# divortio/divortio-lz4

Measured on NVIDIA B200. Metric: lz4_block_roundtrip_throughput, higher is better.
Workload: dtype u8

## Files before the change

divortio-lz4_b200/csrc/api_ctx.inc:

```
namespace {

constexpr int kWarpsFresh16 = 7;
constexpr int kWarpsGeneric32 = 3;
constexpr int kWarpsDecode = 8;
constexpr int kJdGroupEvent = 112;
constexpr int kGtabRegions = 5;
constexpr uint32_t kMaxSplitBlocks = 1u << 20;

struct Buf {
    void *p = nullptr;
    size_t cap = 0;
};

class CopyPool {
  public:
    explicit CopyPool(int threads) {
        for (int i = 0; i < threads; ++i) workers_.emplace_back([this] { run(); });
    }
    ~CopyPool() {
        { std::lock_guard<std::mutex> g(m_); stop_ = true; }
        cv_.notify_all();
        for (std::thread &t : workers_) t.join();
    }
    void copy(void *dst, const void *src, size_t n) {
// ... 50 lines not shown
    std::atomic<size_t> next_{0};
};
constexpr int kSumSlots = 32;
constexpr int kStageSlots = 4;
constexpr size_t kStageBytes = 16u << 20;

}

struct dlz4_ctx {
    int device = 0;
    int sm_count = 0;
    cudaStream_t stream = nullptr, side = nullptr, copy_in = nullptr, copy_out = nullptr;
    cudaStream_t lanes[4] = {};
    uint64_t chunk_bytes = 64ull << 20;
    int n_lanes = 3;
    cudaEvent_t evp[128] = {};
    cudaEvent_t ev0 = nullptr, ev1 = nullptr, ev_side = nullptr, ev_fork = nullptr;
    uint32_t *d_counter = nullptr;
    uint32_t *d_land = nullptr;
    uint32_t *h_one = nullptr;
    uint64_t seg_overlap_min_bytes = 64ull << 20;
    uint32_t *d_hash = nullptr;
    uint64_t *d_total = nullptr;
    int32_t *d_table = nullptr;
    int split = 1;
    bool pw = true;
    int pw_sleep = 200;
    int pw_lead = 7;
    Buf rec;
    uint32_t *d_nrec = nullptr;
    int hybrid = 1;
    int hy_grid = 0;
    int hy_active = 0;
    uint16_t *d_gtabs = nullptr;
    Buf work, comp, seg, out, meta, aux, pin;
    Buf fb_frames, fb_blocks, fb_comp, fb_io;
    std::string last_error;
    uint64_t frame_pipe_min_bytes = 32ull << 20;
    uint64_t jump_min_bytes = 256ull << 10;
    uint64_t seg_min_bytes = 256ull << 10;
    uint32_t seg_jobs = 0, seg_reruns = 0, seg_rounds = 0;
    uint64_t launches = 0;
    float last_ms = 0.f;
    int64_t k_seg_kib = -1, k_seg_warm_kib = -1, k_seg_unit_kib = -1;
    int k_seg_group = -1, k_seg_no_chase = 0, k_jd_unit_mib = 0, k_jd_serial_scan = 0, k_jd_no_overlap = 0, k_debug = 0;
    CopyPool *pool = nullptr;
    int copy_threads = 0;
    uint8_t *stage[kStageSlots] = {};
    cudaEvent_t stage_ev[kStageSlots] = {};
    bool stage_busy[kStageSlots] = {};
    cudaStream_t sum_stream[kSumSlots] = {};
    uint32_t *h_sum = nullptr;
    int probe = 0;
    cudaEvent_t evq[3] = {};
    const uint8_t *res_in = nullptr, *res_out = nullptr;
    uint64_t res_in_len = 0, res_out_len = 0, res_body_len = 0;
};

namespace {

#define CK(call)                                                                                      \
    do {                                                                                              \
        cudaError_t e_ = (call);                                                                      \
        if (e_ != cudaSuccess) {                                                                      \
            char m_[512];                                                                             \
            snprintf(m_, sizeof m_, "%s failed: %s (%s:%d)", #call, cudaGetErrorString(e_), __FILE__, __LINE__); \
            ctx->last_error = m_;                                                                     \
            return DLZ4_E_CUDA;                                                                       \
        }                                                                                             \
    } while (0)

#define CKS(expr)                       \
    do {                                \
        int s_ = (expr);                \
        if (s_ != DLZ4_OK) return s_;   \
    } while (0)

int reserve(dlz4_ctx *ctx, Buf &b, size_t bytes) {
    bytes = (bytes + 255) & ~(size_t)255;
    if (bytes + 256 <= b.cap) return DLZ4_OK;
    if (b.p) CK(cudaFree(b.p));
    b.p = nullptr; b.cap = 0;
    size_t want = bytes + 256;
    CK(cudaMalloc(&b.p, want));
    b.cap = want;
    return DLZ4_OK;
}

int reserve_pinned(dlz4_ctx *ctx, Buf &b, size_t bytes) {
    if (bytes <= b.cap) return DLZ4_OK;
    if (b.p) CK(cudaFreeHost(b.p));
    b.p = nullptr; b.cap = 0;
    CK(cudaMallocHost(&b.p, bytes));
    b.cap = bytes;
    return DLZ4_OK;
}

inline cudaStream_t pick(dlz4_ctx *ctx, void *stream) { return stream ? (cudaStream_t)stream : ctx->stream; }

bool is_pageable(const void *p) {
    cudaPointerAttributes a;
    if (cudaPointerGetAttributes(&a, p) != cudaSuccess) { cudaGetLastError(); return true; }
    return a.type == cudaMemoryTypeUnregistered;
}

int stage_init(dlz4_ctx *ctx) {
    if (ctx->stage[0]) return DLZ4_OK;
// ... 76 lines not shown
```

divortio-lz4_b200/csrc/api_launch.inc:

```
int compress_segmented(dlz4_ctx *ctx, const uint8_t *d_work, int64_t start, int64_t total, int64_t B, uint32_t n, bool linked,
                       const int32_t *init_table, uint8_t *d_comp, const uint64_t *d_coff, uint32_t *d_clen, cudaStream_t st,
                       int32_t *final_table = nullptr, const uint32_t *landed = nullptr, int32_t land_origin = 0,
                       uint32_t land_shift = 0);

int launch_compress(dlz4_ctx *ctx, const uint8_t *src, const uint64_t *src_off, const uint32_t *src_len, uint32_t n,
                    uint32_t max_len, const uint8_t *prefix, uint32_t prefix_len, const int32_t *init_table, uint8_t *dst,
                    const uint64_t *dst_off, uint32_t *comp_len, cudaStream_t st, uint32_t *counter = nullptr, bool dense = false) {
    if (n == 0) return DLZ4_OK;
    if (!counter) counter = ctx->d_counter;
    CK(cudaMemsetAsync(counter, 0, sizeof(uint32_t), st));
    if (init_table == nullptr) { prefix = nullptr; prefix_len = 0; }
    if (max_len <= 65536 && prefix_len == 0 && init_table == nullptr && ctx->split && n <= kMaxSplitBlocks) {
        const size_t region = (size_t)(counter - ctx->d_counter) % kGtabRegions;
        const uint64_t rstride = (uint64_t)max_len / 4 + 2;
        const size_t region_bytes = (((size_t)n * rstride * 8) * 9 / 8 + 255) & ~(size_t)255;
        if (ctx->rec.cap < region_bytes * kGtabRegions + 256) {
            CK(cudaDeviceSynchronize());
            CKS(reserve(ctx, ctx->rec, std::max(region_bytes, (size_t)ctx->rec.cap / kGtabRegions) * kGtabRegions));
        }
        const size_t per_region = ((ctx->rec.cap - 256) / kGtabRegions) & ~(size_t)255;
        uint64_t *recs = (uint64_t *)((uint8_t *)ctx->rec.p + region * per_region);
        uint32_t *nrec = ctx->d_nrec + region * (size_t)kMaxSplitBlocks;
        if (ctx->probe) CK(cudaEventRecord(ctx->evq[0], st));
        if (ctx->pw) {
            const int grid = (int)std::min<uint64_t>(n, (uint64_t)ctx->sm_count);
            const uint32_t lead = (uint32_t)ctx->pw_lead, ns = (uint32_t)ctx->pw_sleep;
            k_parse_pw<<<grid, kPwThreads, kPwSmemBytes, st>>>(src, src_off, src_len, n, recs, rstride, nrec, counter, lead, ns);
        } else
        {
            const int grid = (int)std::min<uint64_t>((n + kWarpsFresh16 - 1) / kWarpsFresh16, (uint64_t)ctx->sm_count);
            k_parse_fresh16<kWarpsFresh16><<<grid, kWarpsFresh16 * 32, kWarpsFresh16 * kHashEntries * 2, st>>>(
                src, src_off, src_len, n, recs, rstride, nrec, counter);
        }
        if (ctx->probe) CK(cudaEventRecord(ctx->evq[1], st));
        CK(cudaMemsetAsync(counter, 0, sizeof(uint32_t), st));
        const int egrid = (int)std::min<uint64_t>((n + kWarpsDecode - 1) / kWarpsDecode, (uint64_t)ctx->sm_count * 8);
        k_encode_blocks<kWarpsDecode><<<egrid, kWarpsDecode * 32, 0, st>>>(src, src_off, src_len, n, recs, rstride, nrec, dst, dst_off,
                                                                            comp_len, counter);
        if (ctx->probe) CK(cudaEventRecord(ctx->evq[2], st));
        ctx->launches++;
    } else if (max_len <= 65536 && prefix_len == 0 && init_table == nullptr && ctx->hybrid) {
        const size_t region = (size_t)(counter - ctx->d_counter) % kGtabRegions;
        const int grid = (int)std::min<uint64_t>(dense ? (n + kHyWarps - 1) / kHyWarps : n, (uint64_t)ctx->hy_grid);
        uint32_t active = dense ? (uint32_t)kHyWarps : (uint32_t)std::min<uint64_t>((n + grid - 1) / grid, (uint64_t)kHyWarps);
        if (ctx->hy_active) active = std::min<uint32_t>(active, (uint32_t)ctx->hy_active);
        k_compress_fresh16h<<<grid, kHyWarps * 32, kHySmemBytes, st>>>(
            src, src_off, src_len, n, dst, dst_off, comp_len, counter,
            ctx->d_gtabs + region * (size_t)ctx->hy_grid * kHyGlWarps * kHashEntries, active);
    } else if (max_len <= 4096 && prefix_len > 0 && init_table != nullptr && ctx->hybrid && prefix_len < 0x7FFF0000u) {
        const size_t region = (size_t)(counter - ctx->d_counter) % kGtabRegions;
        const int grid = (int)std::min<uint64_t>(dense ? (n + kHyWarps - 1) / kHyWarps : n, (uint64_t)ctx->hy_grid);
        const uint32_t active = dense ? (uint32_t)kHyWarps : (uint32_t)std::min<uint64_t>((n + grid - 1) / grid, (uint64_t)kHyWarps);
        k_compress_overlay<<<grid, kHyWarps * 32, kHySmemBytes, st>>>(
            src, src_off, src_len, n, prefix, prefix_len, init_table, dst, dst_off, comp_len, counter,
            ctx->d_gtabs + region * (size_t)ctx->hy_grid * kHyGlWarps * kHashEntries, active);
    } else {
        if (max_len > 65536 && prefix_len == 0 && init_table == nullptr && n <= 65536) {
            std::vector<uint64_t> off(n);
            std::vector<uint32_t> len(n);
            CK(cudaMemcpyAsync(off.data(), src_off, (size_t)n * 8, cudaMemcpyDeviceToHost, st));
            CK(cudaMemcpyAsync(len.data(), src_len, (size_t)n * 4, cudaMemcpyDeviceToHost, st));
            CK(cudaStreamSynchronize(st));
            const uint64_t B = len[0];
            bool uniform = B > 65536 && (B & (B - 1)) == 0 && off[0] + (uint64_t)n * B < 0x7FFFFFF0ull;
            for (uint32_t i = 0; uniform && i < n; ++i)
                uniform = off[i] == off[0] + (uint64_t)i * B && (len[i] == B || (i + 1 == n && len[i] <= B && len[i] > 0));
            if (uniform) {
                const int64_t total = (int64_t)(n - 1) * (int64_t)B + len[n - 1];
                return compress_segmented(ctx, src, (int64_t)off[0], total, (int64_t)B, n, false, nullptr, dst, dst_off, comp_len, st);
            }
        }
        const int grid = (int)std::min<uint64_t>((n + kWarpsGeneric32 - 1) / kWarpsGeneric32, (uint64_t)ctx->sm_count);
        k_compress_generic32<kWarpsGeneric32><<<grid, kWarpsGeneric32 * 32, kWarpsGeneric32 * (kHashEntries * 4 + kRingBytes), st>>>(
            src, src_off, src_len, n, prefix, prefix_len, init_table, dst, dst_off, comp_len, counter);
    }
    ctx->launches++;
    CK(cudaGetLastError());
    return DLZ4_OK;
}

int launch_decompress(dlz4_ctx *ctx, const uint8_t *src, const uint64_t *src_off, const uint32_t *src_len, uint32_t n,
                      uint8_t *dst, const uint64_t *dst_off, const uint32_t *dst_cap, const uint8_t *dict, uint32_t dict_len,
                      int hist_frame, const uint8_t *stored, uint32_t *out_len, uint8_t *status, cudaStream_t st,
                      uint32_t *counter = nullptr) {
    if (n == 0) return DLZ4_OK;
    if (!counter) counter = ctx->d_counter;
    CK(cudaMemsetAsync(counter, 0, sizeof(uint32_t), st));
    const int grid = hist_frame ? 1 : (int)std::min<uint64_t>((n + kWarpsDecode - 1) / kWarpsDecode, (uint64_t)ctx->sm_count * 8);
    if (dict_len)
        k_decompress_blocks<kWarpsDecode, true><<<grid, hist_frame ? 32 : kWarpsDecode * 32, 0, st>>>(src, src_off, src_len, n, dst, dst_off, dst_cap,
                                                                                                      dict, dict_len, hist_frame, stored, out_len, status, counter);
    else
// ... 25 lines not shown
```

divortio-lz4_b200/csrc/api_lifecycle.inc:

```
int dlz4_init(int device, dlz4_ctx **out) {
    if (!out) return DLZ4_E_INVALID_ARG;
    *out = nullptr;
    dlz4_ctx *ctx = new dlz4_ctx();
    ctx->device = device;
    *out = ctx;
    int count = 0;
    CK(cudaGetDeviceCount(&count));
    if (device < 0 || device >= count) { ctx->last_error = "no such CUDA device"; return DLZ4_E_CUDA; }
    CK(cudaSetDevice(device));
    cudaDeviceProp prop;
    CK(cudaGetDeviceProperties(&prop, device));
    ctx->sm_count = prop.multiProcessorCount;
    CK(cudaStreamCreateWithFlags(&ctx->stream, cudaStreamNonBlocking));
    CK(cudaStreamCreateWithFlags(&ctx->side, cudaStreamNonBlocking));
    CK(cudaStreamCreateWithFlags(&ctx->copy_in, cudaStreamNonBlocking));
    CK(cudaStreamCreateWithFlags(&ctx->copy_out, cudaStreamNonBlocking));
    for (cudaEvent_t &e : ctx->evp) CK(cudaEventCreateWithFlags(&e, cudaEventDisableTiming));
    CK(cudaEventCreate(&ctx->ev0));
    CK(cudaEventCreate(&ctx->ev1));
    for (cudaEvent_t &e : ctx->evq) CK(cudaEventCreate(&e));
    CK(cudaEventCreateWithFlags(&ctx->ev_side, cudaEventDisableTiming));
    CK(cudaEventCreateWithFlags(&ctx->ev_fork, cudaEventDisableTiming));
    for (cudaStream_t &l : ctx->lanes) CK(cudaStreamCreateWithFlags(&l, cudaStreamNonBlocking));
    if (const char *e = getenv("DLZ4_SEG_KIB")) ctx->k_seg_kib = std::max(0, atoi(e));
    if (const char *e = getenv("DLZ4_SEG_WARM_KIB")) ctx->k_seg_warm_kib = std::max(0, atoi(e));
    if (const char *e = getenv("DLZ4_SEG_UNIT_KIB")) ctx->k_seg_unit_kib = std::max(0, atoi(e));
    if (const char *e = getenv("DLZ4_SEG_GROUP")) ctx->k_seg_group = std::max(0, atoi(e));
    ctx->k_seg_no_chase = getenv("DLZ4_SEG_NO_CHASE") != nullptr;
    if (const char *e = getenv("DLZ4_JD_UNIT_MIB")) ctx->k_jd_unit_mib = std::max(1, atoi(e));
    ctx->k_jd_serial_scan = getenv("DLZ4_JD_SERIAL_SCAN") != nullptr;
    ctx->k_jd_no_overlap = getenv("DLZ4_JD_NO_OVERLAP") != nullptr;
    ctx->k_debug = getenv("DLZ4_DEBUG") != nullptr;
    if (const char *e = getenv("DLZ4_CHUNK_MIB")) ctx->chunk_bytes = (uint64_t)std::max(1, atoi(e)) << 20;
    if (const char *e = getenv("DLZ4_LANES")) ctx->n_lanes = std::min(4, std::max(1, atoi(e)));
    if (const char *e = getenv("DLZ4_COPY_THREADS")) ctx->copy_threads = std::min(64, std::max(1, atoi(e)));
    CK(cudaMalloc(&ctx->d_counter, 64));
    CK(cudaMalloc(&ctx->d_land, kLandFlags * 4));
    CK(cudaMallocHost(&ctx->h_one, 64));
    *ctx->h_one = 1u;
    if (const char *e = getenv("DLZ4_SEG_OVERLAP_MIN_MIB")) ctx->seg_overlap_min_bytes = (uint64_t)atoll(e) << 20;
    CK(cudaMalloc(&ctx->d_hash, 64));
    CK(cudaMalloc(&ctx->d_total, 64));
    CK(cudaMalloc(&ctx->d_table, kHashEntries * sizeof(int32_t)));
    if (const char *e = getenv("DLZ4_SEG_MIN_KIB")) ctx->seg_min_bytes = (uint64_t)atoll(e) << 10;
    if (const char *e = getenv("DLZ4_JUMP_MIN_KIB")) ctx->jump_min_bytes = (uint64_t)atoll(e) << 10;
    if (const char *e = getenv("DLZ4_SPLIT")) ctx->split = atoi(e) != 0;
    if (const char *e = getenv("DLZ4_PW")) ctx->pw = atoi(e) != 0;
    if (const char *e = getenv("DLZ4_PW_SLEEP")) ctx->pw_sleep = std::max(0, atoi(e));
    if (const char *e = getenv("DLZ4_PW_LEAD")) ctx->pw_lead = std::max(3, std::min(kPwWin - 1, atoi(e)));
    if (const char *e = getenv("DLZ4_HYBRID")) ctx->hybrid = atoi(e) != 0;
    ctx->hy_grid = ctx->sm_count * kHyCtasPerSm;
    if (const char *e = getenv("DLZ4_HY_ACTIVE")) ctx->hy_active = std::max(0, std::min(kHyWarps, atoi(e)));
    CK(cudaMalloc(&ctx->d_gtabs, (size_t)kGtabRegions * ctx->hy_grid * kHyGlWarps * kHashEntries * 2));
    CK(cudaMalloc(&ctx->d_nrec, (size_t)kGtabRegions * kMaxSplitBlocks * 4));
    CK(cudaFuncSetAttribute(k_parse_fresh16<kWarpsFresh16>, cudaFuncAttributeMaxDynamicSharedMemorySize, kWarpsFresh16 * kHashEntries * 2));
    CK(cudaFuncSetAttribute(k_parse_pw, cudaFuncAttributeMaxDynamicSharedMemorySize, kPwSmemBytes));
    CK(cudaFuncSetAttribute(k_compress_fresh16h, cudaFuncAttributeMaxDynamicSharedMemorySize, kHySmemBytes));
    CK(cudaFuncSetAttribute(k_compress_overlay, cudaFuncAttributeMaxDynamicSharedMemorySize, kHySmemBytes));
    CK(cudaFuncSetAttribute(k_compress_segments, cudaFuncAttributeMaxDynamicSharedMemorySize, kSegSmemBytes));
    CK(cudaFuncSetAttribute(k_compress_generic32<kWarpsGeneric32>, cudaFuncAttributeMaxDynamicSharedMemorySize,
                            kWarpsGeneric32 * (kHashEntries * 4 + kRingBytes)));
    CK(cudaFuncSetAttribute(k_compress_chain, cudaFuncAttributeMaxDynamicSharedMemorySize, kHashEntries * 4 + kRingBytes));
    CK(cudaFuncSetAttribute(k_fb_chains, cudaFuncAttributeMaxDynamicSharedMemorySize, kHashEntries * 4 + kRingBytes));
    return DLZ4_OK;
}

void dlz4_shutdown(dlz4_ctx *ctx) {
    if (!ctx) return;
    cudaSetDevice(ctx->device);
    if (ctx->stream) cudaStreamSynchronize(ctx->stream);
    if (ctx->side) cudaStreamSynchronize(ctx->side);
    for (Buf *b : {&ctx->work, &ctx->comp, &ctx->seg, &ctx->out, &ctx->meta, &ctx->aux, &ctx->fb_frames, &ctx->fb_blocks, &ctx->fb_comp, &ctx->fb_io})
        if (b->p) cudaFree(b->p);
    if (ctx->pin.p) cudaFreeHost(ctx->pin.p);
    if (ctx->d_counter) cudaFree(ctx->d_counter);
    if (ctx->d_land) cudaFree(ctx->d_land);
    if (ctx->h_one) cudaFreeHost(ctx->h_one);
    if (ctx->d_hash) cudaFree(ctx->d_hash);
    if (ctx->d_total) cudaFree(ctx->d_total);
    if (ctx->d_table) cudaFree(ctx->d_table);
    if (ctx->d_gtabs) cudaFree(ctx->d_gtabs);
    if (ctx->d_nrec) cudaFree(ctx->d_nrec);
    if (ctx->rec.p) cudaFree(ctx->rec.p);
    delete ctx->pool;
    for (cudaStream_t s : ctx->sum_stream) if (s) { cudaStreamSynchronize(s); cudaStreamDestroy(s); }
    if (ctx->h_sum) cudaFreeHost(ctx->h_sum);
    for (int i = 0; i < kStageSlots; ++i) {
        if (ctx->stage[i]) cudaFreeHost(ctx->stage[i]);
        if (ctx->stage_ev[i]) cudaEventDestroy(ctx->stage_ev[i]);
    }
    if (ctx->ev0) cudaEventDestroy(ctx->ev0);
    if (ctx->ev1) cudaEventDestroy(ctx->ev1);
    for (cudaEvent_t e : ctx->evq) if (e) cudaEventDestroy(e);
    if (ctx->ev_side) cudaEventDestroy(ctx->ev_side);
    if (ctx->ev_fork) cudaEventDestroy(ctx->ev_fork);
    for (cudaEvent_t e : ctx->evp) if (e) cudaEventDestroy(e);
    for (cudaStream_t l : ctx->lanes) if (l) { cudaStreamSynchronize(l); cudaStreamDestroy(l); }
    if (ctx->copy_in) cudaStreamDestroy(ctx->copy_in);
    if (ctx->copy_out) cudaStreamDestroy(ctx->copy_out);
    if (ctx->stream) cudaStreamDestroy(ctx->stream);
    if (ctx->side) cudaStreamDestroy(ctx->side);
    delete ctx;
}

const char *dlz4_strerror(int status) {
    switch (status) {
        case DLZ4_OK: return "ok";
        case DLZ4_E_OUTPUT_TOO_SMALL: return "LZ4: Output Buffer Too Small";
        case DLZ4_E_MALFORMED: return "LZ4: Malformed Input";
        case DLZ4_E_OFFSET_ZERO: return "LZ4: Invalid Offset 0";
        case DLZ4_E_DICT_OOB: return "LZ4: Dictionary Offset Out of Bounds";
        case DLZ4_E_BAD_MAGIC: return "LZ4: Invalid Magic Number";
        case DLZ4_E_BAD_VERSION: return "LZ4: Unsupported Version";
        case DLZ4_E_CONTENT_CHECKSUM: return "LZ4: Content Checksum Error";
        case DLZ4_E_BLOCK_CHECKSUM: return "LZ4: Block Checksum Error";
        case DLZ4_E_HEADER_CHECKSUM: return "LZ4: Header Checksum Error";
        case DLZ4_E_INVALID_ARG: return "dlz4: invalid argument";
        case DLZ4_E_TOO_LARGE: return "dlz4: input of 2 GiB or more in one call";
        case DLZ4_E_CUDA: return "dlz4: CUDA error";
        default: return "dlz4: unknown status";
    }
}

const char *dlz4_last_error(const dlz4_ctx *ctx) { return ctx ? ctx->last_error.c_str() : ""; }
uint64_t dlz4_launch_count(const dlz4_ctx *ctx) { return ctx ? ctx->launches : 0; }
float dlz4_last_kernel_ms(const dlz4_ctx *ctx) { return ctx ? ctx->last_ms : 0.f; }
int dlz4_kernel_probe(dlz4_ctx *ctx, int enable, float *finder_ms, float *encoder_ms) {
    if (!ctx) return DLZ4_E_INVALID_ARG;
    if (finder_ms || encoder_ms) {
        CK(cudaSetDevice(ctx->device));
        CK(cudaEventSynchronize(ctx->evq[2]));
        if (finder_ms) CK(cudaEventElapsedTime(finder_ms, ctx->evq[0], ctx->evq[1]));
        if (encoder_ms) CK(cudaEventElapsedTime(encoder_ms, ctx->evq[1], ctx->evq[2]));
    }
    ctx->probe = enable != 0;
    return DLZ4_OK;
}
void dlz4_segment_stats(const dlz4_ctx *ctx, uint32_t *segments, uint32_t *reruns, uint32_t *rounds) {
    if (segments) *segments = ctx ? ctx->seg_jobs : 0;
    if (reruns) *reruns = ctx ? ctx->seg_reruns : 0;
    if (rounds) *rounds = ctx ? ctx->seg_rounds : 0;
}

uint64_t dlz4_compress_bound(uint64_t n) { return n + n / 255 + 16; }
uint64_t dlz4_frame_bound(uint64_t n) { return 19 + n + (n / 65536 + 1) * 8 + 8 + 64; }

void dlz4_shard_range(uint64_t nblocks, uint32_t world, uint32_t rank, uint64_t *first, uint64_t *count) {
    if (world == 0) world = 1;
    const uint64_t lo = ((uint64_t)rank * nblocks + world - 1) / world;
    const uint64_t hi = ((uint64_t)(rank + 1) * nblocks + world - 1) / world;
    if (first) *first = lo;
    if (count) *count = hi - lo;
}

#ifdef DLZ4_PHASE_TIMING
extern "C" int dlz4_phase_counters(unsigned long long *out16) {
    if (cudaMemcpyFromSymbol(out16, dlz4::g_phase, 16 * sizeof(unsigned long long)) != cudaSuccess) return 1;
    unsigned long long z[16] = {0};
    return cudaMemcpyToSymbol(dlz4::g_phase, z, sizeof z) != cudaSuccess;
}
#endif

void *dlz4_pinned_alloc(uint64_t bytes) {
    void *p = nullptr;
    if (cudaMallocHost(&p, bytes ? bytes : 1) != cudaSuccess) return nullptr;
    return p;
}
void dlz4_pinned_free(void *p) { if (p) cudaFreeHost(p); }
int dlz4_host_register(void *p, uint64_t bytes) {
    if (!p || !bytes) return DLZ4_E_INVALID_ARG;
    return cudaHostRegister(p, (size_t)bytes, cudaHostRegisterPortable | cudaHostRegisterMapped) == cudaSuccess ? DLZ4_OK : (cudaGetLastError(), DLZ4_E_CUDA);
}
int dlz4_host_unregister(void *p) {
    if (!p) return DLZ4_E_INVALID_ARG;
    return cudaHostUnregister(p) == cudaSuccess ? DLZ4_OK : (cudaGetLastError(), DLZ4_E_CUDA);
}
```

divortio-lz4_b200/csrc/dlz4_kernels.cuh:

```cuda
#pragma once
#include <cuda_runtime.h>
#include <stdint.h>
#include <limits.h>

namespace dlz4 {

#ifdef DLZ4_PHASE_TIMING
__device__ unsigned long long g_phase[16];
#define PT_DECL unsigned long long pt_acc[16] = {0,0,0,0,0,0,0,0,0,0,0,0,0,0,0,0}; long long pt_t = clock64();
#define PT_MARK(i) { const long long pt_n = clock64(); pt_acc[i] += (unsigned long long)(pt_n - pt_t); pt_t = pt_n; }
#define PT_COUNT(i, v) { pt_acc[i] += (v); }
#define PT_FLUSH if (lane_id() == 0) { for (int pt_k = 0; pt_k < 16; ++pt_k) atomicAdd(&g_phase[pt_k], pt_acc[pt_k]); }
#define PT_USE(x) asm volatile("" ::"r"((uint32_t)(x)));
#else
#define PT_DECL
#define PT_MARK(i)
#define PT_COUNT(i, v)
#define PT_FLUSH
#define PT_USE(x)
#endif

#ifndef DLZ4_DEC_MINB
#define DLZ4_DEC_MINB 6
#endif
// ... 527 lines not shown
            if (stop) {
                const int l = __ffs(stop) - 1;
                ml = eb + 4 * l + __shfl_sync(FULL, eq, l);
                break;
            }
        }
        if (kEmit) {
            const uint32_t code = (uint32_t)(ml - 4);
            uint8_t *d = emit_literals(out + D, S, anchor, (uint32_t)(s0 - anchor), code < 15u ? code : 15u, lane);
            const uint32_t offset = (uint32_t)(s0 - m0);
            if (lane == 0) { d[0] = (uint8_t)offset; d[1] = (uint8_t)(offset >> 8); }
            d += 2;
            if (code >= 15u) {
                const uint32_t rest = code - 15u, n255 = rest / 255u;
                for (uint32_t i = lane; i < n255; i += 32) d[i] = 255;
                if (lane == 0) d[n255] = (uint8_t)(rest - n255 * 255u);
                d += n255 + 1;
            }
            D = (uint32_t)(d - out);
        }
        pend = 0;
        sIndex = anchor = s0 + ml;
        PT_MARK(8)
        PT_COUNT(11, 1)
        if (s0 >= limit) {
            st.sIndex = sIndex; st.anchor = anchor; st.smc = smc; st.D = D; st.pend = 0; st.head = s0;
            PT_FLUSH
            return kSpanStopped;
        }
    }
    PT_FLUSH
    if (!kEmit) return 0u;
    uint8_t *d = emit_literals(out + D, S, anchor, (uint32_t)(sEnd - anchor), 0u, lane);
    return (uint32_t)(d - out);
}

template <class Tab>
__device__ __forceinline__ uint32_t compress_block_warp_v2(const uint8_t *__restrict__ base, const int32_t start, const int32_t len,
                                                           Tab &T, uint8_t *const out, uint32_t *const ring) {
    SpanState st{start, start, 67u, 0u, 0u, -1};
    return compress_span_warp<Tab, true>(base, start, len, T, out, ring, st, INT_MAX);
}

}
#include "dlz4_wide.cuh"
namespace dlz4 {

__device__ __forceinline__ uint32_t next_block(uint32_t *counter, uint32_t lane) {
    uint32_t b = 0;
    if (lane == 0) b = atomicAdd(counter, 1u);
    return __shfl_sync(FULL, b, 0);
}

}
#include "dlz4_parse.cuh"
#include "dlz4_pw.cuh"
namespace dlz4 {

constexpr int kHyWarps = 7;
constexpr int kHyGlWarps = kHyWarps - 1;
constexpr int kHyCtasPerSm = 4;
constexpr int kHySmemBytes = kHashEntries * 2 + kHyWarps * kRingBytes;
__global__ void __launch_bounds__(kHyWarps * 32, kHyCtasPerSm)
k_compress_fresh16h(const uint8_t *__restrict__ src, const uint64_t *__restrict__ src_off,
                    const uint32_t *__restrict__ src_len, uint32_t nblocks, uint8_t *__restrict__ dst,
                    const uint64_t *__restrict__ dst_off, uint32_t *__restrict__ comp_len, uint32_t *counter,
                    uint16_t *gtabs , uint32_t active_warps) {
    extern __shared__ __align__(16) uint8_t smem[];
    const uint32_t lane = lane_id(), warp = threadIdx.x >> 5;
    if (warp >= active_warps) return;
    uint32_t *ring = reinterpret_cast<uint32_t *>(smem + kHashEntries * 2 + warp * kRingBytes);
    const bool in_smem = warp == 0;
    uint16_t *tab = in_smem ? reinterpret_cast<uint16_t *>(smem)
                            : gtabs + ((size_t)blockIdx.x * kHyGlWarps + (warp - 1)) * kHashEntries;
    uint32_t epoch = 15;
    for (;;) {
        const uint32_t b = next_block(counter, lane);
        if (b >= nblocks) break;
        const uint32_t len = src_len[b];
        if (len > 65536u) { if (lane == 0) comp_len[b] = 0xFFFFFFFFu; continue; }
        uint4 *t4 = reinterpret_cast<uint4 *>(tab);
        const bool small = len <= 4096u;
        if (!small || ++epoch > 15u) {
            if (in_smem) { for (uint32_t i = lane; i < kHashEntries * 2 / 16; i += 32) t4[i] = make_uint4(0, 0, 0, 0); }
            else { for (uint32_t i = lane; i < kHashEntries * 2 / 16; i += 32) __stcg(t4 + i, make_uint4(0, 0, 0, 0)); }
            __syncwarp();
            epoch = small ? 1u : 15u;
        }
        uint32_t c;
        if (small) {
            if (in_smem) { Tab12e<false> T{tab, 0, epoch}; c = compress_block_warp_v2(src + src_off[b], 0, (int32_t)len, T, dst + dst_off[b], ring); }
            else { Tab12e<true> T{tab, 0, epoch}; c = compress_block_warp_v2(src + src_off[b], 0, (int32_t)len, T, dst + dst_off[b], ring); }
        } else if (in_smem) {
            Tab16 T{tab, 0};
            c = compress_block_warp_v2(src + src_off[b], 0, (int32_t)len, T, dst + dst_off[b], ring);
        } else {
            TabG16 T{tab, 0};
            c = compress_block_warp_v2(src + src_off[b], 0, (int32_t)len, T, dst + dst_off[b], ring);
        }
        if (lane == 0) comp_len[b] = c;
        __syncwarp();
    }
}

__global__ void __launch_bounds__(kHyWarps * 32, kHyCtasPerSm)
k_compress_overlay(const uint8_t *__restrict__ src, const uint64_t *__restrict__ src_off, const uint32_t *__restrict__ src_len,
// ... 1504 lines not shown
```

divortio-lz4_b200/csrc/dlz4_parse.cuh:

```cuda
#pragma once

namespace dlz4 {

__device__ __forceinline__ uint2 rec_pack(uint32_t pos, uint32_t ml, uint32_t offset) { return make_uint2(pos | (offset << 16), ml); }

template <class Tab>
__device__ uint32_t parse_block64_warp(const uint8_t *__restrict__ base, const int32_t start, const int32_t len, Tab &T,
                                       uint64_t *__restrict__ rec) {
    const uint32_t lane = lane_id();
    const uint32_t lt = (1u << lane) - 1u;
    const int32_t sEnd = start + len;
    const int32_t mflimit = sEnd - 12;
    const int32_t matchLimit = sEnd - 5;
    int32_t sIndex = start;
    uint32_t smc = 67;
    uint32_t nrec = 0;
    const SrcFlat S{base};

    const uint32_t A0 = (uint32_t)(reinterpret_cast<uintptr_t>(base) & 127u);
    const int32_t wlo = start - (int32_t)((A0 + (uint32_t)start) & 3u);
    const int32_t whi = sEnd;
    uint32_t R0 = 0, R1 = 0, R2 = 0, R3 = 0;
    uint32_t Lc = 0;
    bool cold = true;
    auto load_line = [&](uint32_t l) -> uint32_t {
        const int32_t idx = (int32_t)(l * 128u + 4u * lane) - (int32_t)A0;
        return (idx >= wlo && idx < whi) ? __ldg(reinterpret_cast<const uint32_t *>(base + idx)) : 0u;
    };

    while (sIndex < mflimit) {
        if (smc <= 96u && sIndex + 100 <= sEnd) {
            const int32_t w = sIndex;
            const uint32_t va = A0 + (uint32_t)w;
            const uint32_t wmis = va & 3u;
            const uint32_t L = va >> 7;
            if (cold || L != Lc) {
                const uint32_t d = cold ? 4u : L - Lc;
                if (d == 1u) { R0 = R1; R1 = R2; R2 = R3; R3 = load_line(L + 3u); }
                else if (d == 2u) { R0 = R2; R1 = R3; R2 = load_line(L + 2u); R3 = load_line(L + 3u); }
                else if (d == 3u) { R0 = R3; R1 = load_line(L + 1u); R2 = load_line(L + 2u); R3 = load_line(L + 3u); }
                else { R0 = load_line(L); R1 = load_line(L + 1u); R2 = load_line(L + 2u); R3 = load_line(L + 3u); }
                Lc = L; cold = false;
            }
            const uint32_t wo = ((va & 127u) >> 2) + lane;
            const uint32_t x0 = __shfl_sync(FULL, R0, wo), x1 = __shfl_sync(FULL, R1, wo);
            const uint32_t Tw = wo < 32u ? x0 : x1;
            const uint32_t o = wmis + lane, wi = o >> 2, sh = (o & 3u) * 8u;
            uint32_t Sx[16];
            {
                uint32_t tprev = __shfl_sync(FULL, Tw, wi);
#pragma unroll
                for (int k = 0; k < 16; ++k) {
                    const uint32_t tnext = __shfl_sync(FULL, Tw, wi + k + 1);
                    Sx[k] = __funnelshift_r(tprev, tnext, sh);
                    tprev = tnext;
// ... 138 lines not shown
        const uint32_t prev = same & lt;
        const int j = prev ? 31 - __clz(prev) : (int)lane;
        const int32_t pj = __shfl_sync(FULL, p, j);
        const uint32_t sj = __shfl_sync(FULL, seq, j);
        uint32_t cseq = sj;
        if (prev) cand = pj;
        const bool ok = valid && cand >= 0 && cand != p && (((uint32_t)(p - cand)) >> 16) == 0;
        if (ok && !prev) cseq = S.ld32(cand);
        const bool hit = ok && cseq == seq;
        const uint32_t hits = __ballot_sync(FULL, hit);
        const uint32_t vmask = __ballot_sync(FULL, valid);
        const int hl = __ffs(hits) - 1;
        const uint32_t commit = hits ? ((2u << hl) - 1u) : vmask;
        if (((commit >> lane) & 1u) && ((same & commit) >> lane) == 1u) T.put(h, p);
        __syncwarp();
        if (!hits) {
            if (vmask != FULL) break;
            sIndex += (int32_t)(skip_sum(smc + 32u) - base_sum);
            smc += 32u;
            continue;
        }
        const int32_t s0 = __shfl_sync(FULL, p, hl);
        const int32_t m0 = __shfl_sync(FULL, cand, hl);
        smc = 67;
        int32_t ml;
        for (int32_t eb = 4;; eb += 128) {
            const int32_t q = s0 + eb + 4 * (int32_t)lane;
            int32_t nv = matchLimit - q;
            nv = nv > 4 ? 4 : nv;
            int32_t eq = 0;
            if (nv > 0) {
                const uint32_t x = S.ld32(q) ^ S.ld32(m0 + eb + 4 * (int32_t)lane);
                eq = x ? ((__ffs(x) - 1) >> 3) : 4;
                eq = eq < nv ? eq : nv;
            }
            const uint32_t stop = __ballot_sync(FULL, eq < 4);
            if (stop) {
                const int l = __ffs(stop) - 1;
                ml = eb + 4 * l + __shfl_sync(FULL, eq, l);
                break;
            }
        }
        if (lane == 0) reinterpret_cast<uint2 *>(rec)[nrec] = rec_pack((uint32_t)(s0 - start), (uint32_t)ml, (uint32_t)(s0 - m0));
        ++nrec;
        sIndex = s0 + ml;
    }
    return nrec;
}

template <int WARPS>
__global__ void __launch_bounds__(WARPS * 32, 1)
k_parse_fresh16(const uint8_t *__restrict__ src, const uint64_t *__restrict__ src_off, const uint32_t *__restrict__ src_len,
                uint32_t nblocks, uint64_t *__restrict__ rec_base, uint64_t rec_stride ,
                uint32_t *__restrict__ nrec_out, uint32_t *counter) {
    extern __shared__ __align__(16) uint8_t smem[];
    const uint32_t lane = lane_id(), warp = threadIdx.x >> 5;
    uint16_t *tab = reinterpret_cast<uint16_t *>(smem) + warp * kHashEntries;
    for (;;) {
        const uint32_t b = next_block(counter, lane);
        if (b >= nblocks) break;
        const uint32_t len = src_len[b];
        if (len > 65536u) { if (lane == 0) nrec_out[b] = 0xFFFFFFFFu; continue; }
        uint4 *t4 = reinterpret_cast<uint4 *>(tab);
        for (uint32_t i = lane; i < kHashEntries * 2 / 16; i += 32) t4[i] = make_uint4(0, 0, 0, 0);
        __syncwarp();
        Tab16 T{tab, 0};
        const uint32_t n = parse_block64_warp(src + src_off[b], 0, (int32_t)len, T, rec_base + (uint64_t)b * rec_stride);
        if (lane == 0) nrec_out[b] = n;
        __syncwarp();
    }
}

template <int WARPS>
__global__ void __launch_bounds__(WARPS * 32)
k_encode_blocks(const uint8_t *__restrict__ src, const uint64_t *__restrict__ src_off, const uint32_t *__restrict__ src_len,
                uint32_t nblocks, const uint64_t *__restrict__ rec_base, uint64_t rec_stride, const uint32_t *__restrict__ nrec_in,
                uint8_t *__restrict__ dst, const uint64_t *__restrict__ dst_off, uint32_t *__restrict__ comp_len, uint32_t *counter) {
    const uint32_t lane = lane_id();
    const bool twice = nblocks <= 0x7FFFFFFFu;
    const uint32_t qlen = twice ? 2u * nblocks : nblocks;
    for (;;) {
        const uint32_t qi = next_block(counter, lane);
        if (qi >= qlen) break;
        const uint32_t b = qi < nblocks ? qi : qi - nblocks;
        const uint32_t n = nrec_in[b];
        if (twice && (n != 0xFFFFFFFFu && n >= 256u) != (qi < nblocks)) continue;
        if (n == 0xFFFFFFFFu) { if (lane == 0) comp_len[b] = 0xFFFFFFFFu; continue; }
        const uint8_t *in = src + src_off[b];
        const uint32_t len = src_len[b];
        const uint64_t *rec = rec_base + (uint64_t)b * rec_stride;
        uint8_t *out = dst + dst_off[b];
        uint32_t D = 0, prev_end = 0;
        for (uint32_t r0 = 0; r0 < n; r0 += 32) {
            const uint32_t i = r0 + lane;
            const bool have = i < n;
            const uint2 rc = have ? reinterpret_cast<const uint2 *>(rec)[i] : make_uint2(0u, 0u);
            const uint32_t pos = rc.x & 0xFFFFu, ml = rc.y, offset = rc.x >> 16;
            const uint32_t end = pos + ml;
            uint32_t pe = __shfl_up_sync(FULL, end, 1);
            if (lane == 0) pe = prev_end;
            const uint32_t lit = have ? pos - pe : 0u;
            const uint32_t code = ml - 4u;
            const uint32_t litx = lit >= 15u ? 1u + (lit - 15u) / 255u : 0u;
            const uint32_t mlx = have && code >= 15u ? 1u + (code - 15u) / 255u : 0u;
            const uint32_t size = have ? 3u + litx + lit + mlx : 0u;
            uint32_t incl = size;
#pragma unroll
            for (int o = 1; o < 32; o <<= 1) { const uint32_t y = __shfl_up_sync(FULL, incl, o); if (lane >= (uint32_t)o) incl += y; }
            uint32_t d = D + incl - size;
            if (have) {
                out[d++] = (uint8_t)(((lit < 15u ? lit : 15u) << 4) | (code < 15u ? code : 15u));
                if (lit >= 15u) {
                    uint32_t rest = lit - 15u;
                    while (rest >= 255u) { out[d++] = 255; rest -= 255u; }
                    out[d++] = (uint8_t)rest;
                }
            }
            const uint32_t lits_at = d;
            const bool longrun = have && lit > 24u;
            if (have && !longrun) {
                const uint8_t *s = in + pe;
                for (uint32_t k = 0; k < lit; ++k) out[d + k] = s[k];
            }
            for (uint32_t m = __ballot_sync(FULL, longrun); m; m &= m - 1u) {
                const int l = __ffs(m) - 1;
                const uint32_t o_ = __shfl_sync(FULL, lits_at, l), p_ = __shfl_sync(FULL, pe, l), n_ = __shfl_sync(FULL, lit, l);
                warp_copy(out + o_, in + p_, n_, lane);
            }
            if (have) {
                d += lit;
                out[d] = (uint8_t)offset;
                out[d + 1] = (uint8_t)(offset >> 8);
                d += 2;
                if (code >= 15u) {
                    uint32_t rest = code - 15u;
                    while (rest >= 255u) { out[d++] = 255; rest -= 255u; }
                    out[d] = (uint8_t)rest;
                }
            }
            D += __shfl_sync(FULL, incl, 31);
            const uint32_t last = min(n - r0, 32u) - 1u;
            prev_end = __shfl_sync(FULL, end, last);
        }
        __syncwarp();
        uint8_t *e = emit_literals(out + D, SrcFlat{in}, (int32_t)prev_end, len - prev_end, 0u, lane);
        if (lane == 0) comp_len[b] = (uint32_t)(e - out);
        __syncwarp();
    }
}

}
```

divortio-lz4_b200/csrc/dlz4_pw.cuh:

```cuda
#pragma once

namespace dlz4 {

constexpr int kPwChains = 7;
constexpr int kPwProducers = 2;
constexpr int kPwThreads = 8 * (1 + kPwProducers) * 32;
constexpr int kPwWin = 14;
constexpr uint32_t kPwTmemCols = 128;
constexpr int kPwCtl = 64;
constexpr int kPwChainBytes = kHashEntries * 2 + kPwCtl;
constexpr int kPwSmemBytes = kPwChains * kPwChainBytes + 16;
constexpr uint32_t kPwRingSmc = 160u;
constexpr uint32_t kPwDone = 0x80000000u, kPwSparse = 0x40000000u;
constexpr bool kPwPrefetch = true;
#ifndef DLZ4_PW_CAP
#define DLZ4_PW_CAP 32
#endif
constexpr uint32_t kPwCap = DLZ4_PW_CAP;

struct PwCtl {
    uint32_t w_pos;
    volatile uint32_t block;
    uint32_t ready[kPwWin];
};
// ... 404 lines not shown
            if (pub != v) { pub = v; if (lane == 0) pw_st_release(&ctl->w_pos, pub); }
        }
        const uint32_t base_sum = skip_sum(smc);
        const int32_t p = sIndex + (int32_t)(skip_sum(smc + lane) - base_sum);
        const bool valid = p < mflimit;
        uint32_t seq = 0, h = 0x10000u + lane;
        int32_t cand = -1;
        if (valid) {
            seq = S.ld32(p);
            h = (seq * 2654435761u) >> 18;
            cand = T.get(h);
        }
        const uint32_t same = __match_any_sync(FULL, h);
        const uint32_t prev = same & lt;
        const int j = prev ? 31 - __clz(prev) : (int)lane;
        const int32_t pj = __shfl_sync(FULL, p, j);
        const uint32_t sj = __shfl_sync(FULL, seq, j);
        uint32_t cseq = sj;
        if (prev) cand = pj;
        const bool ok = valid && cand >= 0 && cand != p && (((uint32_t)(p - cand)) >> 16) == 0;
        if (ok && !prev) cseq = S.ld32(cand);
        const bool hit = ok && cseq == seq;
        const uint32_t hits = __ballot_sync(FULL, hit);
        const uint32_t vmask = __ballot_sync(FULL, valid);
        const int hl = __ffs(hits) - 1;
        const uint32_t commit = hits ? ((2u << hl) - 1u) : vmask;
        if (((commit >> lane) & 1u) && ((same & commit) >> lane) == 1u) T.put(h, p);
        __syncwarp();
        if (!hits) {
            if (vmask != FULL) break;
            sIndex += (int32_t)(skip_sum(smc + 32u) - base_sum);
            smc += 32u;
            PT_MARK(3) PT_COUNT(12, 1)
            continue;
        }
        const int32_t s0 = __shfl_sync(FULL, p, hl);
        const int32_t m0 = __shfl_sync(FULL, cand, hl);
        smc = 67;
        const uint32_t ml = pw_extend(base, s0, m0, 4, matchLimit, lane);
        if (lane == 0) rec2[nrec] = rec_pack((uint32_t)s0, ml, (uint32_t)(s0 - m0));
        ++nrec;
        sIndex = s0 + (int32_t)ml;
        PT_MARK(3) PT_COUNT(12, 1)
    }
    PT_MARK(5)
    PT_FLUSH
    return nrec;
}

__global__ void __launch_bounds__(kPwThreads, 1)
k_parse_pw(const uint8_t *__restrict__ src, const uint64_t *__restrict__ src_off, const uint32_t *__restrict__ src_len,
           uint32_t nblocks, uint64_t *__restrict__ rec_base, uint64_t rec_stride ,
           uint32_t *__restrict__ nrec_out, uint32_t *counter, uint32_t lead,
           uint32_t full_ns ) {
    extern __shared__ __align__(16) uint8_t smem[];
    constexpr uint32_t kRoles = 1 + kPwProducers;
    constexpr uint32_t kTeam = kRoles * 32;
    const uint32_t lane = lane_id(), warp = threadIdx.x >> 5;
    const uint32_t quarter = warp & 3u, tslot = (warp >> 2) / kRoles, role = (warp >> 2) % kRoles;
    const uint32_t chain = quarter + 4u * tslot;
    uint32_t *const taddr_smem = reinterpret_cast<uint32_t *>(smem + kPwChains * kPwChainBytes);
    if (warp == 0) {
        asm volatile("tcgen05.alloc.cta_group::1.sync.aligned.shared::cta.b32 [%0], %1;\n\t"
                     "tcgen05.relinquish_alloc_permit.cta_group::1.sync.aligned;"
                     ::"r"((uint32_t)__cvta_generic_to_shared(taddr_smem)), "r"(kPwTmemCols) : "memory");
    }
    tm_fence_before();
    __syncthreads();
    tm_fence_after();
    const uint32_t taddr = *taddr_smem;
    const uint32_t tcol = taddr + ((32u * quarter) << 16) + tslot * (uint32_t)(kPwWin * 4);
    if (chain < (uint32_t)kPwChains) {
        const uint32_t tid = role * 32u + lane;
        uint8_t *const cb = smem + (size_t)chain * kPwChainBytes;
        uint16_t *const tab = reinterpret_cast<uint16_t *>(cb);
        PwCtl *const ctl = reinterpret_cast<PwCtl *>(cb + kHashEntries * 2);
        const uint32_t bar = 1u + chain;
        uint32_t first = chain * gridDim.x + blockIdx.x;
        const uint32_t qbase = gridDim.x * (uint32_t)kPwChains;
        bool have_first = true;
        for (;;) {
            pw_bar(bar, kTeam);
            if (role == 0 && lane == 0) {
                uint32_t b;
                if (have_first) b = first; else b = qbase + atomicAdd(counter, 1u);
                ctl->block = b < nblocks ? b : 0xFFFFFFFFu;
                ctl->w_pos = 0u;
            }
            have_first = false;
            pw_bar(bar, kTeam);
            const uint32_t b = ctl->block;
            if (b == 0xFFFFFFFFu) break;
            const uint32_t len = src_len[b];
            if (len > 65536u) {
                if (role == 0 && lane == 0) nrec_out[b] = 0xFFFFFFFFu;
                continue;
            }
            {
                uint4 *z = reinterpret_cast<uint4 *>(cb);
                for (uint32_t i = tid; i < kHashEntries * 2 / 16; i += kTeam) z[i] = make_uint4(0, 0, 0, 0);
                if (tid < (uint32_t)kPwWin) ctl->ready[tid] = 0u;
            }
            pw_bar(bar, kTeam);
            const uint8_t *base = src + src_off[b];
            uint64_t *const rec = rec_base + (uint64_t)b * rec_stride;
            const uint32_t nwin = len >= 112u ? (len - 111u) / 32u + 1u : 0u;
            if (role == 0) {
                const uint32_t n = pw_walker(base, (int32_t)len, nwin, tab, tcol, ctl, rec, lane);
                if (lane == 0) {
                    nrec_out[b] = n;
                    pw_st_release(&ctl->w_pos, kPwDone);
                }
            } else {
                pw_producer(base, nwin, lead, role - 1u, tab, tcol, ctl, lane, full_ns);
            }
        }
    }
    tm_fence_before();
    __syncthreads();
    tm_fence_after();
    if (warp == 0)
        asm volatile("tcgen05.dealloc.cta_group::1.sync.aligned.b32 %0, %1;" ::"r"(taddr), "r"(kPwTmemCols) : "memory");
}

}
```

Baseline: 78.62.

## Overlap parse and encode kernels via PDL with per-block readiness flags

Launches the encode kernel with programmatic stream serialization so it can start while the parse kernel is still running. The parse kernel publishes each block's record count with release stores, and encode CTAs poll those flags with acquire loads, claiming blocks by CAS over three passes. The passes are large ready blocks, then any ready block, then a blocking wait. Encoding also moves from one warp per block to a whole CTA per block, with warps splitting records and a shared-memory prefix of sizes. Probe timing switches from events to globaltimer atomics. The change risks spin-waiting, deadlock if parse CTAs cannot be scheduled (guarded by a trap), and extra memsets per launch.

```diff
diff --git a/divortio-lz4_b200/csrc/api_ctx.inc b/divortio-lz4_b200/csrc/api_ctx.inc
--- a/divortio-lz4_b200/csrc/api_ctx.inc
+++ b/divortio-lz4_b200/csrc/api_ctx.inc
@@ -126,7 +126,8 @@
     cudaStream_t sum_stream[kSumSlots] = {};
     uint32_t *h_sum = nullptr;
     int probe = 0;
-    cudaEvent_t evq[3] = {};
+    unsigned long long *d_tprobe = nullptr;
+    cudaEvent_t ev_probe = nullptr;
     const uint8_t *res_in = nullptr, *res_out = nullptr;
     uint64_t res_in_len = 0, res_out_len = 0, res_body_len = 0;
 };
diff --git a/divortio-lz4_b200/csrc/api_launch.inc b/divortio-lz4_b200/csrc/api_launch.inc
--- a/divortio-lz4_b200/csrc/api_launch.inc
+++ b/divortio-lz4_b200/csrc/api_launch.inc
@@ -21,23 +21,38 @@
         const size_t per_region = ((ctx->rec.cap - 256) / kGtabRegions) & ~(size_t)255;
         uint64_t *recs = (uint64_t *)((uint8_t *)ctx->rec.p + region * per_region);
         uint32_t *nrec = ctx->d_nrec + region * (size_t)kMaxSplitBlocks;
-        if (ctx->probe) CK(cudaEventRecord(ctx->evq[0], st));
+        uint32_t *ecounter = ctx->d_counter + 11 + region;
+        CK(cudaMemsetAsync(ecounter, 0, sizeof(uint32_t), st));
+        CK(cudaMemsetAsync(nrec, kNrecPending & 0xFF, (size_t)n * 4, st));
+        unsigned long long *tprobe = nullptr;
+        if (ctx->probe) {
+            tprobe = ctx->d_tprobe;
+            CK(cudaMemsetAsync(tprobe, 0xFF, 2 * sizeof(unsigned long long), st));
+            CK(cudaMemsetAsync(tprobe + 2, 0, 2 * sizeof(unsigned long long), st));
+        }
         if (ctx->pw) {
             const int grid = (int)std::min<uint64_t>(n, (uint64_t)ctx->sm_count);
             const uint32_t lead = (uint32_t)ctx->pw_lead, ns = (uint32_t)ctx->pw_sleep;
-            k_parse_pw<<<grid, kPwThreads, kPwSmemBytes, st>>>(src, src_off, src_len, n, recs, rstride, nrec, counter, lead, ns);
+            k_parse_pw<<<grid, kPwThreads, kPwSmemBytes, st>>>(src, src_off, src_len, n, recs, rstride, nrec, counter, lead, ns, tprobe);
         } else
         {
             const int grid = (int)std::min<uint64_t>((n + kWarpsFresh16 - 1) / kWarpsFresh16, (uint64_t)ctx->sm_count);
             k_parse_fresh16<kWarpsFresh16><<<grid, kWarpsFresh16 * 32, kWarpsFresh16 * kHashEntries * 2, st>>>(
-                src, src_off, src_len, n, recs, rstride, nrec, counter);
+                src, src_off, src_len, n, recs, rstride, nrec, counter, tprobe);
         }
-        if (ctx->probe) CK(cudaEventRecord(ctx->evq[1], st));
-        CK(cudaMemsetAsync(counter, 0, sizeof(uint32_t), st));
-        const int egrid = (int)std::min<uint64_t>((n + kWarpsDecode - 1) / kWarpsDecode, (uint64_t)ctx->sm_count * 8);
-        k_encode_blocks<kWarpsDecode><<<egrid, kWarpsDecode * 32, 0, st>>>(src, src_off, src_len, n, recs, rstride, nrec, dst, dst_off,
-                                                                            comp_len, counter);
-        if (ctx->probe) CK(cudaEventRecord(ctx->evq[2], st));
+        cudaLaunchConfig_t cfg = {};
+        cudaLaunchAttribute attr[1];
+        attr[0].id = cudaLaunchAttributeProgrammaticStreamSerialization;
+        attr[0].val.programmaticStreamSerializationAllowed = 1;
+        cfg.gridDim = dim3((unsigned)std::min<uint64_t>(n, (uint64_t)ctx->sm_count * 8));
+        cfg.blockDim = dim3(kWarpsDecode * 32);
+        cfg.dynamicSmemBytes = 0;
+        cfg.stream = st;
+        cfg.attrs = attr;
+        cfg.numAttrs = 1;
+        CK(cudaLaunchKernelEx(&cfg, k_encode_blocks<kWarpsDecode>, src, src_off, src_len, n, (const uint64_t *)recs, rstride, nrec, dst,
+                              dst_off, comp_len, ecounter, tprobe));
+        if (ctx->probe) CK(cudaEventRecord(ctx->ev_probe, st));
         ctx->launches++;
     } else if (max_len <= 65536 && prefix_len == 0 && init_table == nullptr && ctx->hybrid) {
         const size_t region = (size_t)(counter - ctx->d_counter) % kGtabRegions;
diff --git a/divortio-lz4_b200/csrc/api_lifecycle.inc b/divortio-lz4_b200/csrc/api_lifecycle.inc
--- a/divortio-lz4_b200/csrc/api_lifecycle.inc
+++ b/divortio-lz4_b200/csrc/api_lifecycle.inc
@@ -18,7 +18,7 @@
     for (cudaEvent_t &e : ctx->evp) CK(cudaEventCreateWithFlags(&e, cudaEventDisableTiming));
     CK(cudaEventCreate(&ctx->ev0));
     CK(cudaEventCreate(&ctx->ev1));
-    for (cudaEvent_t &e : ctx->evq) CK(cudaEventCreate(&e));
+    CK(cudaEventCreateWithFlags(&ctx->ev_probe, cudaEventDisableTiming));
     CK(cudaEventCreateWithFlags(&ctx->ev_side, cudaEventDisableTiming));
     CK(cudaEventCreateWithFlags(&ctx->ev_fork, cudaEventDisableTiming));
     for (cudaStream_t &l : ctx->lanes) CK(cudaStreamCreateWithFlags(&l, cudaStreamNonBlocking));
@@ -35,6 +35,7 @@
     if (const char *e = getenv("DLZ4_LANES")) ctx->n_lanes = std::min(4, std::max(1, atoi(e)));
     if (const char *e = getenv("DLZ4_COPY_THREADS")) ctx->copy_threads = std::min(64, std::max(1, atoi(e)));
     CK(cudaMalloc(&ctx->d_counter, 64));
+    CK(cudaMalloc(&ctx->d_tprobe, 4 * sizeof(unsigned long long)));
     CK(cudaMalloc(&ctx->d_land, kLandFlags * 4));
     CK(cudaMallocHost(&ctx->h_one, 64));
     *ctx->h_one = 1u;
@@ -74,6 +75,7 @@
         if (b->p) cudaFree(b->p);
     if (ctx->pin.p) cudaFreeHost(ctx->pin.p);
     if (ctx->d_counter) cudaFree(ctx->d_counter);
+    if (ctx->d_tprobe) cudaFree(ctx->d_tprobe);
     if (ctx->d_land) cudaFree(ctx->d_land);
     if (ctx->h_one) cudaFreeHost(ctx->h_one);
     if (ctx->d_hash) cudaFree(ctx->d_hash);
@@ -91,7 +93,7 @@
     }
     if (ctx->ev0) cudaEventDestroy(ctx->ev0);
     if (ctx->ev1) cudaEventDestroy(ctx->ev1);
-    for (cudaEvent_t e : ctx->evq) if (e) cudaEventDestroy(e);
+    if (ctx->ev_probe) cudaEventDestroy(ctx->ev_probe);
     if (ctx->ev_side) cudaEventDestroy(ctx->ev_side);
     if (ctx->ev_fork) cudaEventDestroy(ctx->ev_fork);
     for (cudaEvent_t e : ctx->evp) if (e) cudaEventDestroy(e);
@@ -129,9 +131,11 @@
     if (!ctx) return DLZ4_E_INVALID_ARG;
     if (finder_ms || encoder_ms) {
         CK(cudaSetDevice(ctx->device));
-        CK(cudaEventSynchronize(ctx->evq[2]));
-        if (finder_ms) CK(cudaEventElapsedTime(finder_ms, ctx->evq[0], ctx->evq[1]));
-        if (encoder_ms) CK(cudaEventElapsedTime(encoder_ms, ctx->evq[1], ctx->evq[2]));
+        CK(cudaEventSynchronize(ctx->ev_probe));
+        unsigned long long t[4];
+        CK(cudaMemcpy(t, ctx->d_tprobe, sizeof(t), cudaMemcpyDeviceToHost));
+        if (finder_ms) *finder_ms = (float)((double)(t[2] - t[0]) * 1e-6);
+        if (encoder_ms) *encoder_ms = (float)((double)(t[3] - t[1]) * 1e-6);
     }
     ctx->probe = enable != 0;
     return DLZ4_OK;
diff --git a/divortio-lz4_b200/csrc/dlz4_kernels.cuh b/divortio-lz4_b200/csrc/dlz4_kernels.cuh
--- a/divortio-lz4_b200/csrc/dlz4_kernels.cuh
+++ b/divortio-lz4_b200/csrc/dlz4_kernels.cuh
@@ -603,6 +603,20 @@
     return __shfl_sync(FULL, b, 0);
 }
 
+__device__ __forceinline__ uint32_t ld_acquire_gpu(const uint32_t *p) {
+    uint32_t v;
+    asm volatile("ld.acquire.gpu.global.u32 %0, [%1];" : "=r"(v) : "l"(p) : "memory");
+    return v;
+}
+__device__ __forceinline__ void st_release_gpu(uint32_t *p, const uint32_t v) {
+    asm volatile("st.release.gpu.global.u32 [%0], %1;" ::"l"(p), "r"(v) : "memory");
+}
+__device__ __forceinline__ uint64_t globaltimer_ns() {
+    uint64_t t;
+    asm volatile("mov.u64 %0, %%globaltimer;" : "=l"(t));
+    return t;
+}
+
 }
 #include "dlz4_parse.cuh"
 #include "dlz4_pw.cuh"
diff --git a/divortio-lz4_b200/csrc/dlz4_parse.cuh b/divortio-lz4_b200/csrc/dlz4_parse.cuh
--- a/divortio-lz4_b200/csrc/dlz4_parse.cuh
+++ b/divortio-lz4_b200/csrc/dlz4_parse.cuh
@@ -1,6 +1,9 @@
 #pragma once
 
 namespace dlz4 {
+
+constexpr uint32_t kNrecPending = 0xFEFEFEFEu;
+constexpr uint32_t kNrecTaken = 0xFEFEFEFDu;
 
 __device__ __forceinline__ uint2 rec_pack(uint32_t pos, uint32_t ml, uint32_t offset) { return make_uint2(pos | (offset << 16), ml); }
 
@@ -245,58 +248,97 @@
 __global__ void __launch_bounds__(WARPS * 32, 1)
 k_parse_fresh16(const uint8_t *__restrict__ src, const uint64_t *__restrict__ src_off, const uint32_t *__restrict__ src_len,
                 uint32_t nblocks, uint64_t *__restrict__ rec_base, uint64_t rec_stride ,
-                uint32_t *__restrict__ nrec_out, uint32_t *counter) {
+                uint32_t *__restrict__ nrec_out, uint32_t *counter, unsigned long long *tprobe ) {
     extern __shared__ __align__(16) uint8_t smem[];
     const uint32_t lane = lane_id(), warp = threadIdx.x >> 5;
     uint16_t *tab = reinterpret_cast<uint16_t *>(smem) + warp * kHashEntries;
+    if (tprobe && threadIdx.x == 0) atomicMin(&tprobe[0], globaltimer_ns());
     for (;;) {
         const uint32_t b = next_block(counter, lane);
         if (b >= nblocks) break;
         const uint32_t len = src_len[b];
-        if (len > 65536u) { if (lane == 0) nrec_out[b] = 0xFFFFFFFFu; continue; }
+        if (len > 65536u) { if (lane == 0) st_release_gpu(&nrec_out[b], 0xFFFFFFFFu); continue; }
         uint4 *t4 = reinterpret_cast<uint4 *>(tab);
         for (uint32_t i = lane; i < kHashEntries * 2 / 16; i += 32) t4[i] = make_uint4(0, 0, 0, 0);
         __syncwarp();
         Tab16 T{tab, 0};
         const uint32_t n = parse_block64_warp(src + src_off[b], 0, (int32_t)len, T, rec_base + (uint64_t)b * rec_stride);
-        if (lane == 0) nrec_out[b] = n;
         __syncwarp();
+        if (lane == 0) st_release_gpu(&nrec_out[b], n);
     }
-}
+    if (tprobe && lane == 0) atomicMax(&tprobe[2], globaltimer_ns());
+}
+
+__device__ __forceinline__ uint32_t seq_size(const uint2 rc, const uint32_t pe) {
+    const uint32_t pos = rc.x & 0xFFFFu, code = rc.y - 4u, lit = pos - pe;
+    return 3u + (lit >= 15u ? 1u + (lit - 15u) / 255u : 0u) + lit + (code >= 15u ? 1u + (code - 15u) / 255u : 0u);
+}
+__device__ __forceinline__ uint32_t rec_end(const uint2 rc) { return (rc.x & 0xFFFFu) + rc.y; }
 
 template <int WARPS>
 __global__ void __launch_bounds__(WARPS * 32)
 k_encode_blocks(const uint8_t *__restrict__ src, const uint64_t *__restrict__ src_off, const uint32_t *__restrict__ src_len,
-                uint32_t nblocks, const uint64_t *__restrict__ rec_base, uint64_t rec_stride, const uint32_t *__restrict__ nrec_in,
-                uint8_t *__restrict__ dst, const uint64_t *__restrict__ dst_off, uint32_t *__restrict__ comp_len, uint32_t *counter) {
-    const uint32_t lane = lane_id();
-    const bool twice = nblocks <= 0x7FFFFFFFu;
-    const uint32_t qlen = twice ? 2u * nblocks : nblocks;
+                uint32_t nblocks, const uint64_t *__restrict__ rec_base, uint64_t rec_stride, uint32_t *nrec,
+                uint8_t *__restrict__ dst, const uint64_t *__restrict__ dst_off, uint32_t *__restrict__ comp_len, uint32_t *counter,
+                unsigned long long *tprobe ) {
+    __shared__ uint32_t s_qi, s_n, s_size[WARPS];
+    const uint32_t lane = lane_id(), warp = threadIdx.x >> 5;
+    if (tprobe && threadIdx.x == 0) atomicMin(&tprobe[1], globaltimer_ns());
     for (;;) {
-        const uint32_t qi = next_block(counter, lane);
-        if (qi >= qlen) break;
-        const uint32_t b = qi < nblocks ? qi : qi - nblocks;
-        const uint32_t n = nrec_in[b];
-        if (twice && (n != 0xFFFFFFFFu && n >= 256u) != (qi < nblocks)) continue;
-        if (n == 0xFFFFFFFFu) { if (lane == 0) comp_len[b] = 0xFFFFFFFFu; continue; }
+        __syncthreads();
+        if (threadIdx.x == 0) {
+            const uint32_t qi = atomicAdd(counter, 1u);
+            uint32_t n = kNrecTaken;
+            if (qi < 3u * nblocks) {
+                const uint32_t pass = qi / nblocks, b = qi - pass * nblocks;
+                uint32_t v = ld_acquire_gpu(&nrec[b]);
+                if (pass == 2 && v == kNrecPending) {
+                    const long long t0 = clock64();
+                    do {
+                        __nanosleep(256);
+                        if (clock64() - t0 > (8ll << 30)) __trap();
+                        v = ld_acquire_gpu(&nrec[b]);
+                    } while (v == kNrecPending);
+                }
+                const bool take = v != kNrecPending && v != kNrecTaken && (pass != 0 || (v != 0xFFFFFFFFu && v >= 256u));
+                if (take && atomicCAS(&nrec[b], v, kNrecTaken) == v) n = v;
+            }
+            s_qi = qi;
+            s_n = n;
+        }
+        __syncthreads();
+        const uint32_t qi = s_qi, n = s_n;
+        if (qi >= 3u * nblocks) break;
+        if (n == kNrecTaken) continue;
+        const uint32_t b = qi % nblocks;
+        if (n == 0xFFFFFFFFu) { if (threadIdx.x == 0) comp_len[b] = 0xFFFFFFFFu; continue; }
         const uint8_t *in = src + src_off[b];
         const uint32_t len = src_len[b];
-        const uint64_t *rec = rec_base + (uint64_t)b * rec_stride;
+        const uint2 *rec = reinterpret_cast<const uint2 *>(rec_base + (uint64_t)b * rec_stride);
         uint8_t *out = dst + dst_off[b];
-        uint32_t D = 0, prev_end = 0;
-        for (uint32_t r0 = 0; r0 < n; r0 += 32) {
+        const uint32_t per = ((n + WARPS - 1) / WARPS + 31u) & ~31u;
+        const uint32_t lo = min(n, warp * per), hi = min(n, lo + per);
+        const uint32_t start_end = lo ? rec_end(rec[lo - 1]) : 0u;
+        {
+            uint32_t sz = 0;
+            for (uint32_t i = lo + lane; i < hi; i += 32) sz += seq_size(rec[i], i ? rec_end(rec[i - 1]) : 0u);
+            sz = __reduce_add_sync(FULL, sz);
+            if (lane == 0) s_size[warp] = sz;
+        }
+        __syncthreads();
+        uint32_t D = 0, prev_end = start_end;
+        for (uint32_t w = 0; w < warp; ++w) D += s_size[w];
+        for (uint32_t r0 = lo; r0 < hi; r0 += 32) {
             const uint32_t i = r0 + lane;
-            const bool have = i < n;
-            const uint2 rc = have ? reinterpret_cast<const uint2 *>(rec)[i] : make_uint2(0u, 0u);
+            const bool have = i < hi;
+            const uint2 rc = have ? rec[i] : make_uint2(0u, 0u);
             const uint32_t pos = rc.x & 0xFFFFu, ml = rc.y, offset = rc.x >> 16;
             const uint32_t end = pos + ml;
             uint32_t pe = __shfl_up_sync(FULL, end, 1);
             if (lane == 0) pe = prev_end;
             const uint32_t lit = have ? pos - pe : 0u;
             const uint32_t code = ml - 4u;
-            const uint32_t litx = lit >= 15u ? 1u + (lit - 15u) / 255u : 0u;
-            const uint32_t mlx = have && code >= 15u ? 1u + (code - 15u) / 255u : 0u;
-            const uint32_t size = have ? 3u + litx + lit + mlx : 0u;
+            const uint32_t size = have ? seq_size(rc, pe) : 0u;
             uint32_t incl = size;
 #pragma unroll
             for (int o = 1; o < 32; o <<= 1) { const uint32_t y = __shfl_up_sync(FULL, incl, o); if (lane >= (uint32_t)o) incl += y; }
@@ -332,14 +374,17 @@
                 }
             }
             D += __shfl_sync(FULL, incl, 31);
-            const uint32_t last = min(n - r0, 32u) - 1u;
+            const uint32_t last = min(hi - r0, 32u) - 1u;
             prev_end = __shfl_sync(FULL, end, last);
         }
-        __syncwarp();
-        uint8_t *e = emit_literals(out + D, SrcFlat{in}, (int32_t)prev_end, len - prev_end, 0u, lane);
-        if (lane == 0) comp_len[b] = (uint32_t)(e - out);
-        __syncwarp();
+        if (warp == WARPS - 1) {
+            __syncwarp();
+            uint8_t *e = emit_literals(out + D, SrcFlat{in}, (int32_t)prev_end, len - prev_end, 0u, lane);
+            if (lane == 0) comp_len[b] = (uint32_t)(e - out);
+        }
     }
-}
-
-}
+    if (tprobe && threadIdx.x == 0) atomicMax(&tprobe[3], globaltimer_ns());
+    asm volatile("griddepcontrol.wait;" ::: "memory");
+}
+
+}
diff --git a/divortio-lz4_b200/csrc/dlz4_pw.cuh b/divortio-lz4_b200/csrc/dlz4_pw.cuh
--- a/divortio-lz4_b200/csrc/dlz4_pw.cuh
+++ b/divortio-lz4_b200/csrc/dlz4_pw.cuh
@@ -480,8 +480,10 @@
 k_parse_pw(const uint8_t *__restrict__ src, const uint64_t *__restrict__ src_off, const uint32_t *__restrict__ src_len,
            uint32_t nblocks, uint64_t *__restrict__ rec_base, uint64_t rec_stride ,
            uint32_t *__restrict__ nrec_out, uint32_t *counter, uint32_t lead,
-           uint32_t full_ns ) {
+           uint32_t full_ns ,
+           unsigned long long *tprobe ) {
     extern __shared__ __align__(16) uint8_t smem[];
+    if (tprobe && threadIdx.x == 0) atomicMin(&tprobe[0], globaltimer_ns());
     constexpr uint32_t kRoles = 1 + kPwProducers;
     constexpr uint32_t kTeam = kRoles * 32;
     const uint32_t lane = lane_id(), warp = threadIdx.x >> 5;
@@ -518,10 +520,13 @@
             have_first = false;
             pw_bar(bar, kTeam);
             const uint32_t b = ctl->block;
-            if (b == 0xFFFFFFFFu) break;
+            if (b == 0xFFFFFFFFu) {
+                asm volatile("griddepcontrol.launch_dependents;" ::: "memory");
+                break;
+            }
             const uint32_t len = src_len[b];
             if (len > 65536u) {
-                if (role == 0 && lane == 0) nrec_out[b] = 0xFFFFFFFFu;
+                if (role == 0 && lane == 0) st_release_gpu(&nrec_out[b], 0xFFFFFFFFu);
                 continue;
             }
             {
@@ -535,8 +540,9 @@
             const uint32_t nwin = len >= 112u ? (len - 111u) / 32u + 1u : 0u;
             if (role == 0) {
                 const uint32_t n = pw_walker(base, (int32_t)len, nwin, tab, tcol, ctl, rec, lane);
+                __syncwarp();
                 if (lane == 0) {
-                    nrec_out[b] = n;
+                    st_release_gpu(&nrec_out[b], n);
                     pw_st_release(&ctl->w_pos, kPwDone);
                 }
             } else {
@@ -549,6 +555,7 @@
     tm_fence_after();
     if (warp == 0)
         asm volatile("tcgen05.dealloc.cta_group::1.sync.aligned.b32 %0, %1;" ::"r"(taddr), "r"(kPwTmemCols) : "memory");
-}
-
-}
+    if (tprobe && threadIdx.x == 0) atomicMax(&tprobe[2], globaltimer_ns());
+}
+
+}
```

Result: slower. 74.87, median of 6 (-4.8%).
